# mit-acl/rl_collision_avoidance

Hardware: AMD Instinct MI355X
Metric: agent-steps/sec (env.step) at 4 agents x 8192 worlds per GPU (higher is better)
Workload: dtype f64

## Files before the change

### include/cavoid.h

```cpp
#ifndef CAVOID_H
#define CAVOID_H
#include <stdint.h>

#ifdef __cplusplus
extern "C" {
#endif

#define CAVOID_ABI_VERSION 3
#define CAVOID_MAX_ACTIONS 32
#define CAVOID_MAX_AGENTS 64

#define CAVOID_F_AT_GOAL 0x01u
#define CAVOID_F_RAN_OUT 0x02u
#define CAVOID_F_IN_COLL 0x04u
#define CAVOID_F_WAS_AT_GOAL 0x08u
#define CAVOID_F_WAS_IN_COLL 0x10u
#define CAVOID_F_PRESENT 0x20u
#define CAVOID_F_LEARNING 0x40u
#define CAVOID_F_POLICY_SHIFT 8
#define CAVOID_F_POLICY_MASK 7u
enum { CAVOID_POLICY_EXTERNAL = 0, CAVOID_POLICY_STATIC = 1, CAVOID_POLICY_NONCOOP = 2, CAVOID_POLICY_RVO = 3, CAVOID_POLICY_FROZEN_NET = 4 };
#define CAVOID_F_DONE_MASK 0x07u

enum { CAVOID_SORT_CLOSEST_LAST = 0, CAVOID_SORT_CLOSEST_FIRST = 1, CAVOID_SORT_TIME_TO_IMPACT = 2 };
// ... 95 lines not shown

enum {
    CAVOID_FORM_NONE = 0,
    CAVOID_FORM_STEP = 1,
    CAVOID_FORM_QUAD = 2,
    CAVOID_FORM_RVO = 3,
    CAVOID_FORM_LOOP_PF = 4,
    CAVOID_FORM_LOOP = 5,
    CAVOID_FORM_PIPE = 6,
    CAVOID_FORM_RELAY = 7,
    CAVOID_FORM_CROWD = 8,
    CAVOID_FORM_CROWD_RVO = 9
};
int32_t cavoid_last_step_form(const cavoid_env *env, int32_t *relay_consumers);

int cavoid_step_continuous_autoreset(cavoid_env *env, const float *actions , float *obs, float *rewards, uint8_t *done,
                                     uint8_t *game_over, void *stream);
int cavoid_step_continuous_autoreset_n(cavoid_env *env, const float *actions, int64_t action_stride, int32_t n_steps, int64_t out_step_stride,
                                       float *obs, float *rewards, uint8_t *done, uint8_t *game_over, void *stream);

int32_t cavoid_packed_width(const cavoid_env *env);
int cavoid_reset_packed(cavoid_env *env, const uint8_t *world_mask, float *packed, void *stream);
int cavoid_observe_packed(cavoid_env *env, float *packed, void *stream);
int cavoid_step_packed(cavoid_env *env, const int32_t *actions, float *packed, uint8_t *game_over, void *stream);
int cavoid_step_autoreset_packed(cavoid_env *env, const int32_t *actions, int64_t action_stride, int32_t n_steps, int64_t out_step_stride,
                                 float *packed, uint8_t *game_over, void *stream);
int cavoid_step_continuous_autoreset_packed(cavoid_env *env, const float *actions, int64_t action_stride, int32_t n_steps,
                                            int64_t out_step_stride, float *packed, uint8_t *game_over, void *stream);

typedef struct cavoid_comm cavoid_comm;
// ... 133 lines not shown
```

### rl_collision_avoidance_amd/_lib.py

```python
from __future__ import annotations

import ctypes as C
import os

from .build import LIB_PATH as _DEFAULT_LIB_PATH

LIB_PATH = os.environ.get("CAVOID_LIB", _DEFAULT_LIB_PATH)

MAX_ACTIONS = 32
MAX_AGENTS = 64
TILE_MAX_AGENTS = 16
RVO_WAVE = 2
ABI_VERSION = 3

F_AT_GOAL, F_RAN_OUT, F_IN_COLL, F_WAS_AT_GOAL, F_WAS_IN_COLL, F_PRESENT, F_LEARNING = 1, 2, 4, 8, 16, 32, 64
F_POLICY_SHIFT = 8
F_POLICY_MASK = 7
POLICY_EXTERNAL, POLICY_STATIC, POLICY_NONCOOP, POLICY_RVO, POLICY_FROZEN_NET = 0, 1, 2, 3, 4
F_DONE_MASK = 7
COMM_FORCE_RCCL = 1
STEP_FORMS = ("NONE", "STEP", "QUAD", "RVO", "LOOP_PF", "LOOP", "PIPE", "RELAY", "CROWD", "CROWD_RVO")


class CavoidCfg(C.Structure):
# ... 54 lines not shown
        self.code = code


_P = C.c_void_p
SYMBOLS = [
    ("cavoid_abi_version", C.c_int, []),
    ("cavoid_strerror", C.c_char_p, [C.c_int]),
    ("cavoid_last_hip_error", C.c_int, []),
    ("cavoid_default_cfg", C.c_int, [C.POINTER(CavoidCfg), C.c_int32, C.c_int32]),
    ("cavoid_default_actions", C.c_int, [_P, C.POINTER(C.c_int32)]),
    ("cavoid_create", C.c_int, [C.POINTER(CavoidCfg), C.c_int64, C.c_int64, C.c_int, C.POINTER(_P)]),
    ("cavoid_destroy", None, [_P]),
    ("cavoid_num_worlds", C.c_int64, [_P]),
    ("cavoid_obs_width", C.c_int32, [_P]),
    ("cavoid_last_step_form", C.c_int32, [_P, C.POINTER(C.c_int32)]),
    ("cavoid_seed", C.c_int, [_P, C.c_uint64, _P, _P]),
    ("cavoid_get_episode", C.c_int, [_P, _P, _P]),
    ("cavoid_pool_refresh", C.c_int, [_P, C.c_uint32, _P]),
    ("cavoid_set_state", C.c_int, [_P, _P, _P, _P, _P]),
    ("cavoid_get_state", C.c_int, [_P, _P, _P, _P, _P]),
    ("cavoid_reset", C.c_int, [_P, _P, _P, _P]),
    ("cavoid_observe", C.c_int, [_P, _P, _P]),
    ("cavoid_step", C.c_int, [_P, _P, _P, _P, _P, _P, _P]),
    ("cavoid_step_continuous", C.c_int, [_P, _P, _P, _P, _P, _P, _P]),
    ("cavoid_step_autoreset", C.c_int, [_P, _P, _P, _P, _P, _P, _P]),
    ("cavoid_step_autoreset_n", C.c_int, [_P, _P, C.c_int64, C.c_int32, C.c_int64, _P, _P, _P, _P, _P]),
    ("cavoid_step_continuous_autoreset", C.c_int, [_P, _P, _P, _P, _P, _P, _P]),
    ("cavoid_step_continuous_autoreset_n", C.c_int, [_P, _P, C.c_int64, C.c_int32, C.c_int64, _P, _P, _P, _P, _P]),
    ("cavoid_step_continuous_autoreset_packed", C.c_int, [_P, _P, C.c_int64, C.c_int32, C.c_int64, _P, _P, _P]),
    ("cavoid_step_autoreset_n_timed", C.c_int, [_P, _P, C.c_int64, C.c_int32, C.c_int32, C.c_int64, _P, _P, _P, _P, _P, C.POINTER(C.c_float)]),
# ... 77 lines not shown
```

### rl_collision_avoidance_amd/batched_env.py

```python
from __future__ import annotations

import ctypes as C
from typing import Optional, Tuple

import numpy as np
import torch

from . import _lib
from .config import EnvConfig

_SORT = {"closest_last": 0, "closest_first": 1, "time_to_impact": 2}
_DYN = {"unicycle": 0, "unicycle_max_turn_rate": 1, "holonomic": 2}


def make_cfg(config: Optional[EnvConfig] = None, **overrides) -> _lib.CavoidCfg:
    config = config or EnvConfig()
    cfg = _lib.CavoidCfg()
    N = int(config.MAX_NUM_AGENTS_IN_ENVIRONMENT)
    M = int(config.MAX_NUM_OTHER_AGENTS_OBSERVED)
    _lib.check(_lib.lib().cavoid_default_cfg(C.byref(cfg), N, M), "cavoid_default_cfg")
    cfg.dt = config.DT
    cfg.near_goal_threshold = config.NEAR_GOAL_THRESHOLD
    cfg.max_time_ratio = config.MAX_TIME_RATIO
    cfg.collision_dist = config.COLLISION_DIST
# ... 181 lines not shown
    def refresh_pool(self, epoch: int) -> None:
        _lib.check(self._lib.cavoid_pool_refresh(self._h, int(epoch) & 0xFFFFFFFF, self._stream()), "cavoid_pool_refresh")

    @property
    def episode(self) -> torch.Tensor:
        out = torch.empty((self.num_worlds,), dtype=torch.int32, device=self.device)
        _lib.check(self._lib.cavoid_get_episode(self._h, self._ptr(out), self._stream()), "cavoid_get_episode")
        return out

    @property
    def last_step_form(self) -> Tuple[str, int]:
        nc = C.c_int32(0)
        form = self._lib.cavoid_last_step_form(self._h, C.byref(nc))
        return _lib.STEP_FORMS[form], int(nc.value)

    def set_state(self, state_f64: torch.Tensor, state_f32: torch.Tensor, flags: torch.Tensor) -> None:
        A = self.num_worlds * self.max_agents
        f64 = self._want(state_f64, (4, A), torch.float64, "state_f64")
        f32 = self._want(state_f32, (5, A), torch.float32, "state_f32")
        fl = self._want(flags, (A,), torch.int32, "flags")
        _lib.check(self._lib.cavoid_set_state(self._h, self._ptr(f64), self._ptr(f32), self._ptr(fl), self._stream()),
                   "cavoid_set_state")

    def get_state(self) -> Tuple[torch.Tensor, torch.Tensor, torch.Tensor]:
        A = self.num_worlds * self.max_agents
        f64 = torch.empty((4, A), dtype=torch.float64, device=self.device)
        f32 = torch.empty((5, A), dtype=torch.float32, device=self.device)
        fl = torch.empty((A,), dtype=torch.int32, device=self.device)
        _lib.check(self._lib.cavoid_get_state(self._h, self._ptr(f64), self._ptr(f32), self._ptr(fl), self._stream()),
                   "cavoid_get_state")
# ... 164 lines not shown
```

### rl_collision_avoidance_amd/csrc/cavoid_capi.hip

```cpp
#include <hip/hip_runtime.h>
#include <hip/hip_ext.h>

#include <cmath>
#include <cstdlib>
#include <cstring>
#include <new>

#include "cavoid.h"
#include "cavoid_host.hpp"
#include "cavoid_kernels.hpp"
#include "cavoid_launch.hpp"
#include "cavoid_crowd.hpp"

using namespace cavoid;

thread_local int g_last_hip_error = 0;

extern "C" int cavoid_abi_version(void) { return CAVOID_ABI_VERSION; }

extern "C" int cavoid_last_hip_error(void) { return g_last_hip_error; }

extern "C" const char *cavoid_strerror(int code) {
    switch (code) {
        case CAVOID_OK: return "ok";
// ... 313 lines not shown
        return cavoid_launch_rvo(e, MODE, io, s, ev_start, ev_stop);
    if (MODE == MODE_STEP_AUTORESET) {
        const int rc = cavoid_launch_quad(e, io, s, ev_start, ev_stop);
        if (rc != CAVOID_EUNSUPPORTED) return rc;
    }
    const int rc = launch_on<MODE>(e, e->k, e->st, e->grid, io, s, ev_start, ev_stop);
    return stepping ? note_form(e, rc, CAVOID_FORM_STEP) : rc;
}

extern "C" int32_t cavoid_last_step_form(const cavoid_env *e, int32_t *relay_consumers) {
    const int32_t form = e ? e->last_form : CAVOID_FORM_NONE;
    if (relay_consumers) *relay_consumers = form == CAVOID_FORM_RELAY ? e->last_relay_consumers : 0;
    return form;
}

int cavoid_ahead_prepare(cavoid_env *e, int32_t n_steps, hipStream_t s, hipEvent_t *timed_start) {
    if (!e || e->ahead_R <= 0) return CAVOID_OK;
    if (n_steps + 1 > e->ahead_R) return CAVOID_EUNSUPPORTED;
    hipStreamCaptureStatus cap = hipStreamCaptureStatusNone;
    (void)hipStreamIsCapturing(s, &cap);
    const bool capturing = cap != hipStreamCaptureStatusNone;
    if (capturing) e->ahead_always = true;
    if (!e->ahead_always && e->ahead_primed && e->ahead_budget >= n_steps + 1) return CAVOID_OK;
    const int64_t waves = (e->W + e->k.wpw - 1) / e->k.wpw;
    const bool in_place = e->ahead_always;
    const dim3 grid((unsigned)((waves + 3) / 4), in_place ? 1u : (e->ahead_primed ? 4u : 32u)), block(256);
    const uint32_t *hi_in = e->ahead_hi[e->ahead_cur];
    uint32_t *hi_out = e->ahead_hi[in_place ? e->ahead_cur : (e->ahead_cur ^ 1)];
    hipEvent_t ev_fill = (timed_start && !capturing) ? *timed_start : nullptr;
    if (ev_fill) *timed_start = nullptr;
    const int rc = dispatch_n(e->cfg.max_agents, EnvNs{}, [&](auto n) -> int {
        launch_kernel(ahead_fill_kernel<decltype(n)::value>, grid, block, 0, s, ev_fill, nullptr, e->k, e->st.episode, hi_in, hi_out, e->pool, e->ahead_R);
        return CAVOID_OK;
    });
    if (rc != CAVOID_OK) return rc;
    HIP_TRY(hipGetLastError());
    if (!in_place) e->ahead_cur ^= 1;
    if (!capturing) { e->ahead_primed = true; e->ahead_budget = e->ahead_R; }
    return CAVOID_OK;
}
void cavoid_ahead_consumed(cavoid_env *e, int32_t n_steps) {
    if (!e || e->ahead_R <= 0) return;
    e->ahead_budget = e->ahead_budget > n_steps ? e->ahead_budget - n_steps : 0;
}

static int fill_pool(cavoid_env *e, hipStream_t s) {
    if (e->ahead_R > 0) {
        e->ahead_budget = 0;
        e->ahead_primed = false;
        HIP_TRY(hipMemsetAsync(e->ahead_hi[0], 0xFF, 2 * (size_t)e->W * sizeof(uint32_t), s));
        return CAVOID_OK;
    }
    if (e->pool_size <= 0) return CAVOID_OK;
    HIP_TRY(hipMemsetAsync(e->pool_episode, 0xFF, (size_t)e->pool_size * sizeof(uint32_t), s));
    KCfg k = e->k;
    k.num_worlds = e->pool_size;
    k.world_offset = 0;
    k.pool_size = 0;
// ... 119 lines not shown
    return launch<MODE_STEP>(e, io, static_cast<hipStream_t>(stream));
}

static int launch_autoreset(cavoid_env *e, KIO io, const int32_t *actions, int64_t action_stride, int32_t n_steps, int64_t out_step_stride,
                            hipStream_t s, hipEvent_t ev_start = nullptr, hipEvent_t ev_stop = nullptr, const float *cont = nullptr) {
    if (e->cfg.dynamics == CAVOID_DYN_HOLONOMIC && !cont) return CAVOID_EINVAL;
    if (n_steps < 1 || action_stride < 0) return CAVOID_EINVAL;
    if (cont && n_steps > 1 && action_stride != 0 && action_stride < 2 * e->A) return CAVOID_EINVAL;
    if (out_step_stride != 0 && out_step_stride < e->W) return CAVOID_EINVAL;
    io.out_step_stride = n_steps > 1 ? out_step_stride : 0;
    io.actions = actions;
    io.cont = cont;
    io.action_stride = action_stride;
    io.n_steps = n_steps;
    e->last_form = CAVOID_FORM_NONE;
    if (int rc = cavoid_ahead_prepare(e, n_steps, s, &ev_start)) return rc;
    const int rc = (n_steps > 1 || e->prefetch_single)
                       ? cavoid_launch_multistep(e, io, e->latency_mode != 0, s, ev_start, ev_stop)
                       : launch<MODE_STEP_AUTORESET>(e, io, s, ev_start, ev_stop);
    cavoid_ahead_consumed(e, n_steps);
    return rc;
}

extern "C" int cavoid_step_autoreset(cavoid_env *e, const int32_t *actions, float *obs, float *rew, uint8_t *done, uint8_t *game_over, void *stream) {
    if (step_args(e, actions, rew, done, game_over) != CAVOID_OK) return CAVOID_EINVAL;
    return launch_autoreset(e, plain_io(e, obs, rew, done, game_over), actions, 0, 1, 0, static_cast<hipStream_t>(stream));
}

extern "C" int cavoid_step_autoreset_n(cavoid_env *e, const int32_t *actions, int64_t action_stride, int32_t n_steps, int64_t out_step_stride,
                                       float *obs, float *rew, uint8_t *done, uint8_t *game_over, void *stream) {
    if (step_args(e, actions, rew, done, game_over) != CAVOID_OK || n_steps < 0) return CAVOID_EINVAL;
    if (n_steps == 0) return CAVOID_OK;
    return launch_autoreset(e, plain_io(e, obs, rew, done, game_over), actions, action_stride, n_steps, out_step_stride,
                            static_cast<hipStream_t>(stream));
}
// ... 118 lines not shown
```

### rl_collision_avoidance_amd/csrc/cavoid_kernels.hpp

```cpp
#pragma once
#include <hip/hip_runtime.h>
#include <stdint.h>

#include "cavoid.h"

namespace cavoid {

#ifdef CAVOID_TRACE
__device__ unsigned long long *g_trace = nullptr;
#define CAVOID_STAMP(k)                                                                \
    do {                                                                               \
        if (lane == 0 && g_trace) g_trace[wave * 16 + (k)] = (unsigned long long)clock64(); \
    } while (0)
#else
#define CAVOID_STAMP(k) do { } while (0)
#endif

#define CAVOID_RARE(x) __builtin_expect(!!(x), 0)
#ifndef CAVOID_SKIP
#define CAVOID_SKIP 0
#endif

constexpr double kPi = 3.14159265358979323846;
constexpr int kTileMaxAgents = 16;
// ... 53 lines not shown

struct KIO {
    PoolRec *pool_out;
    const int32_t *actions;
    const float *cont;
    const uint8_t *mask;
    float *obs;
    float *rew;
    uint8_t *done;
    uint8_t *game_over;
    int64_t action_stride;
    int64_t out_step_stride;
    int32_t n_steps;
    int32_t obs_stride;
    int32_t packed;
};

__device__ __forceinline__ double wrap_closed_fixup(double a, uint32_t switches) {
    if (CAVOID_RARE(switches & kSwWrapClosed)) a = a == -kPi ? kPi : a;
    return a;
}
__device__ __forceinline__ double wrap_angle(double a, uint32_t switches) {
    a = a >= kPi ? a - 2.0 * kPi : a;
    a = a < -kPi ? a + 2.0 * kPi : a;
    if (CAVOID_RARE(__ballot(a >= kPi || a < -kPi) != 0ull)) {
        while (a >= kPi) a -= 2.0 * kPi;
        while (a < -kPi) a += 2.0 * kPi;
    }
    return wrap_closed_fixup(a, switches);
}
// ... 684 lines not shown
    a.gx = r.gx; a.gy = r.gy; a.radius = r.radius; a.pref = r.pref;
    a.flags = r.flags;
    a.vx = a.vy = 0.0;
    a.speed = 0.0f;
}

template <int N>
__device__ __forceinline__ void new_episode(const KCfg &c, const PoolRec *pool, uint32_t gw, uint32_t ep, int i, Agent &a) {
    if (c.pool_size > 0) {
        load_pool(pool, (int64_t)pool_index(c, gw, ep) * N + i, a);
    } else {
        generate_agent<N>(c, gw, ep, i, a);
    }
}

template <int N>
__device__ __forceinline__ void ahead_fill_wave(const KCfg &c, const uint32_t *episode, const uint32_t *hi_in, uint32_t *hi_out, PoolRec *ahead, const int need,
                                                const int64_t wave, const int lane, const int y, const int ny, double *sc_d, float *sc_r) {
    const int wpw = c.wpw, lanes_used = wpw * N;
    const int lw = lane / N, i = lane - lw * N;
    const int64_t w = wave * wpw + lw;
    const bool active = lane < lanes_used && w < c.num_worlds;
    const int base = lane < lanes_used ? lw * N : 0;
    uint32_t ep = 0u, fh = 0u;
    if (active) {
        ep = episode[w];
        fh = hi_in[w];
        if (fh == 0xFFFFFFFFu || (int32_t)(fh - ep) < 0) fh = ep;
    }
    const uint32_t target = ep + (uint32_t)need;
    int missing = active ? (int)(int32_t)(target - fh) : 0;
    missing = missing < 0 ? 0 : missing;
    int trips = missing;
#pragma unroll
    for (int o = 32; o > 0; o >>= 1) { const int v = __shfl_xor(trips, o, 64); trips = v > trips ? v : trips; }
    const uint32_t gw = (uint32_t)(c.world_offset + w);
    for (int k = y; k < trips; k += ny) {
        const uint32_t e = fh + 1u + (uint32_t)k;
        const bool fresh = active && k < missing;
        Agent a;
        absent_agent(a);
        if (c.gen_mode == 1) generate_world_v2<N>(c, gw, e, i, base, lane, fresh, sc_d, sc_d + 64, sc_d + 128, sc_d + 192, sc_r, a);
        else if (fresh) generate_agent<N>(c, gw, e, i, a);
        if (fresh) {
            PoolRec r;
            r.px = a.px; r.py = a.py; r.heading = a.heading; r.t_rem = a.t_rem;
            r.gx = a.gx; r.gy = a.gy; r.radius = a.radius; r.pref = a.pref;
            r.flags = a.flags; r.pad[0] = r.pad[1] = r.pad[2] = 0u;
            ahead[((int64_t)w * c.ahead + (int64_t)(e & (uint32_t)(c.ahead - 1))) * N + i] = r;
        }
    }
    if (active && i == 0 && y == 0) hi_out[w] = missing > 0 ? target : fh;
}

template <int N>
__global__ void __launch_bounds__(256) ahead_fill_kernel(const KCfg c, const uint32_t *episode, const uint32_t *hi_in, uint32_t *hi_out, PoolRec *ahead, const int need) {
    __shared__ double sh_d[4][4 * 64];
    __shared__ float sh_r[4][64];
    const int wave_in_block = threadIdx.x >> 6;
    ahead_fill_wave<N>(c, episode, hi_in, hi_out, ahead, need, (int64_t)blockIdx.x * 4 + wave_in_block, threadIdx.x & 63, (int)blockIdx.y, (int)gridDim.y,
                       sh_d[wave_in_block], sh_r[wave_in_block]);
}

constexpr double kRvoEps = 1e-5;
__device__ __forceinline__ double det2(double ax, double ay, double bx, double by) { return ax * by - ay * bx; }

struct Line { double px, py, dx, dy; };
// ... 731 lines not shown
```

### rl_collision_avoidance_amd/csrc/cavoid_launch.hpp

```cpp
#pragma once
#include <hip/hip_runtime.h>
#include <hip/hip_ext.h>

#include <type_traits>

#include "cavoid.h"
#include "cavoid_host.hpp"
#include "cavoid_kernels.hpp"

struct cavoid_env {
    int device = 0;
    int64_t W = 0, A = 0, world_offset = 0;
    cavoid_cfg cfg{};
    cavoid::KCfg k{};
    cavoid::KState st{};
    cavoid::PoolRec *pool = nullptr;
    uint32_t *pool_episode = nullptr;
    int64_t pool_size = 0;
    int ahead_R = 0;
    uint32_t *ahead_hi[2] = {nullptr, nullptr};
    int ahead_cur = 0;
    int ahead_budget = 0;
    bool ahead_primed = false;
    bool ahead_always = false;
    void *slab = nullptr;
    void *pool_slab = nullptr;
    double *d_actions = nullptr;
    int waves_per_block = 4;
    int grid = 0;
    int pipeline = 2;
    int relay_consumers = 3;
    int latency_mode = 0;
    int quad = -1;
    int prefetch_single = 0;
    int last_form = CAVOID_FORM_NONE;
    int last_relay_consumers = 0;
    hipEvent_t ev0 = nullptr, ev1 = nullptr;
};

// ... 80 lines not shown
    const dim3 grid((unsigned)tiles), block(128);
    const int rc = dispatch_n(e->cfg.max_agents, EnvNs{}, [&](auto n) -> int {
        constexpr int N = decltype(n)::value;
        const size_t lds = pipe_lds_fixed_bytes<N>() + tail;
        if (lds > 65536) return CAVOID_EUNSUPPORTED;
        launch_kernel(env_pipe_kernel<N, RVO>, grid, block, lds, s, ev_start, ev_stop, k, e->st, e->pool, io);
        return CAVOID_OK;
    });
    if (rc != CAVOID_OK) return rc;
    HIP_TRY(hipGetLastError());
    return CAVOID_OK;
}

}

int cavoid_ahead_prepare(cavoid_env *e, int32_t n_steps, hipStream_t s, hipEvent_t *timed_start = nullptr);
void cavoid_ahead_consumed(cavoid_env *e, int32_t n_steps);
int cavoid_launch_relay(cavoid_env *e, const cavoid::KIO &io, hipStream_t s, hipEvent_t ev_start, hipEvent_t ev_stop);
int cavoid_launch_quad(cavoid_env *e, const cavoid::KIO &io, hipStream_t s, hipEvent_t ev_start, hipEvent_t ev_stop);
int cavoid_launch_multistep(cavoid_env *e, const cavoid::KIO &io, bool prefetch, hipStream_t s, hipEvent_t ev_start, hipEvent_t ev_stop);
int cavoid_launch_rvo(cavoid_env *e, int mode, const cavoid::KIO &io, hipStream_t s, hipEvent_t ev_start, hipEvent_t ev_stop);
int cavoid_launch_crowd(cavoid_env *e, int mode, const cavoid::KCfg &k, const cavoid::KState &st, int64_t worlds, const cavoid::KIO &io,
                        hipStream_t s, hipEvent_t ev_start, hipEvent_t ev_stop);
int cavoid_launch_crowd_rvo(cavoid_env *e, int mode, const cavoid::KCfg &k, const cavoid::KState &st, int64_t worlds, const cavoid::KIO &io,
                            hipStream_t s, hipEvent_t ev_start, hipEvent_t ev_stop);
static inline int crowd_step_form(const cavoid_env *e) { return e->k.rvo_enabled ? CAVOID_FORM_CROWD_RVO : CAVOID_FORM_CROWD; }
#ifdef CAVOID_TRACE
int cavoid_debug_trace_multistep(unsigned long long *dev_ptr);
int cavoid_debug_trace_rvo(unsigned long long *dev_ptr);
int cavoid_debug_trace_relay(unsigned long long *dev_ptr);
int cavoid_debug_trace_quad(unsigned long long *dev_ptr);
#endif
```

### rl_collision_avoidance_amd/csrc/cavoid_multistep.hip

```cpp
#include "cavoid_launch.hpp"

using namespace cavoid;

int cavoid_launch_multistep(cavoid_env *e, const KIO &io, bool prefetch, hipStream_t s, hipEvent_t ev_start, hipEvent_t ev_stop) {
    if (crowd_form(e->cfg.max_agents))
        return note_form(e, cavoid_launch_crowd(e, MODE_STEP_AUTORESET_N, e->k, e->st, e->W, io, s, ev_start, ev_stop), crowd_step_form(e));
    if (e->k.rvo_enabled || (e->k.gen_mode == 1 && e->k.pool_size <= 0))
        return cavoid_launch_rvo(e, prefetch ? MODE_STEP_AUTORESET_PF : MODE_STEP_AUTORESET_N, io, s, ev_start, ev_stop);
    if (prefetch && e->pipeline >= 2 && !io.cont) {
        const int rc = cavoid_launch_relay(e, io, s, ev_start, ev_stop);
        if (rc != CAVOID_EUNSUPPORTED) return rc;
    }
    if (prefetch && e->pipeline && !io.cont) {
        const int rc = launch_pipe<false>(e, io, s, ev_start, ev_stop);
        if (rc != CAVOID_EUNSUPPORTED) return note_form(e, rc, CAVOID_FORM_PIPE);
    }
    if (prefetch) return note_form(e, launch_on<MODE_STEP_AUTORESET_PF>(e, e->k, e->st, e->grid, io, s, ev_start, ev_stop), CAVOID_FORM_LOOP_PF);
    return note_form(e, launch_on<MODE_STEP_AUTORESET_N>(e, e->k, e->st, e->grid, io, s, ev_start, ev_stop), CAVOID_FORM_LOOP);
}

#ifdef CAVOID_TRACE
int cavoid_debug_trace_multistep(unsigned long long *dev_ptr) { return set_trace(dev_ptr); }
#endif
```

### rl_collision_avoidance_amd/csrc/cavoid_relay.hip

```cpp
#include "cavoid_launch.hpp"
#include "cavoid_relay.hpp"

using namespace cavoid;

template <int N>
static int relay_allow_lds() {
    static bool allowed = false;
    if (!allowed) {
        HIP_TRY(hipFuncSetAttribute(reinterpret_cast<const void *>(env_relay_kernel<N>), hipFuncAttributeMaxDynamicSharedMemorySize, (int)kRelayLdsLimit));
        allowed = true;
    }
    return CAVOID_OK;
}

int cavoid_launch_relay(cavoid_env *e, const KIO &io, hipStream_t s, hipEvent_t ev_start, hipEvent_t ev_stop) {
    const KCfg &k = e->k;
    if (k.rvo_enabled || k.pool_size <= 0 || !io.obs || !io.actions || io.cont) return CAVOID_EUNSUPPORTED;
    if (k.switches & kSwSkipDonePairs) return CAVOID_EUNSUPPORTED;
    const int64_t tiles = (e->W + k.wpw - 1) / k.wpw;
    if (tiles > 512) return CAVOID_EUNSUPPORTED;
    if (e->cfg.max_agents > kRelayMaxAgents) return CAVOID_EUNSUPPORTED;
    const int row = io.obs_stride;
    const int tile_floats = (k.tile_rows * row + 3) & ~3;
    if (k.tile_rows < k.wpw * e->cfg.max_agents) return CAVOID_EUNSUPPORTED;
    const dim3 grid((unsigned)tiles);
    int used_nc = 0;
    const int rc = dispatch_n(e->cfg.max_agents, RelayNs{}, [&](auto n) -> int {
        constexpr int N = decltype(n)::value;
        int nc = e->relay_consumers;
        while (nc > 1 && relay_lds_fixed_bytes<N>() + (size_t)nc * tile_floats * sizeof(float) > kRelayLdsLimit) --nc;
        const size_t lds = relay_lds_fixed_bytes<N>() + (size_t)nc * tile_floats * sizeof(float);
        if (lds > kRelayLdsLimit || (nc < 2 && e->relay_consumers >= 2)) return CAVOID_EUNSUPPORTED;
        if (lds > 65536) {
            const int rc_opt = relay_allow_lds<N>();
            if (rc_opt != CAVOID_OK) return rc_opt;
        }
        used_nc = nc;
        launch_kernel(env_relay_kernel<N>, grid, dim3(64 * (3 + nc)), lds, s, ev_start, ev_stop, k, e->st, e->pool, io);
        return CAVOID_OK;
    });
    if (rc != CAVOID_OK) return rc;
    HIP_TRY(hipGetLastError());
    return note_form(e, CAVOID_OK, CAVOID_FORM_RELAY, used_nc);
}

#ifdef CAVOID_TRACE
int cavoid_debug_trace_relay(unsigned long long *dev_ptr) { return set_trace(dev_ptr); }
#endif
```

### rl_collision_avoidance_amd/csrc/cavoid_relay.hpp

```cpp
#pragma once
#include "cavoid_kernels.hpp"

namespace cavoid {

constexpr int kRelayMaxAgents = 6;
template <int N>
__host__ __device__ constexpr int relay_ring() { return N <= 5 ? 8 : 4; }
constexpr size_t kRelayLdsLimit = 80 * 1024;
constexpr int kRelayActRing = 64;
constexpr int kRelayActAhead = 48;
constexpr int kRelayEvq = 8;

struct RelaySeq {
    int spec;
    int stage;
    int res;
    int fin;
    int act;
    int ev;
    int nxt;
    int cons[kRelayMaxConsumers];
    int cfin[kRelayMaxConsumers];
    int coop[2];
    int kernarg[2];
    int tile_id;
};
static_assert(sizeof(RelaySeq) % 16 == 0, "the event queue behind it holds 64-bit masks; the tiles further on are read 16 bytes at a time");
struct RelayTent { double px[64], py[64], vx[64], vy[64], heading[64]; float r[64], gx[64], gy[64], pref[64]; uint32_t flags[64]; };
struct RelayRes { uint32_t flags[64], ctl[64]; float rew[64]; };
struct RelayNxt { double px[64], py[64], heading[64], t_rem[64]; float gx[64], gy[64], radius[64], pref[64]; uint32_t flags[64]; };
#ifndef CAVOID_RELAY_ORDER
#define CAVOID_RELAY_ORDER 0x432150
#endif
#ifndef CAVOID_RELAY_PRIO_D
#define CAVOID_RELAY_PRIO_D 3
#endif
#ifndef CAVOID_RELAY_PRIO_P
#define CAVOID_RELAY_PRIO_P 3
#endif
#ifndef CAVOID_RELAY_PRIO_L
#define CAVOID_RELAY_PRIO_L 0
#endif
#ifndef CAVOID_RELAY_PRIO_C
#define CAVOID_RELAY_PRIO_C 1
#endif
#ifndef CAVOID_RELAY_ABL
#define CAVOID_RELAY_ABL 0
#endif
__device__ __forceinline__ int relay_role_of(int wv, int NC) {
    if (NC == 3) return (int)(((unsigned)CAVOID_RELAY_ORDER >> (4 * wv)) & 15u);
    return wv;
}
constexpr int kRelayCoopWaves = 3;
constexpr int kRelayCoopFromN = 4;
template <int N>
struct RelayCoop {
    static constexpr int K = Others<N>::K;
    uint64_t key[K][64];
    uint32_t bits[K][64];
// ... 197 lines not shown
#endif
        uint32_t lo = orderable((float)(ry * e.tx - rx * e.ty));
        if (SW) {
            if (c.switches & kSwIndexTie) lo = (uint32_t)other_index(st.i, o, N);
            if (c.switches & kSwExactGap) { lo = 0u; hi = 0x7FFFFFFEu - (orderable((float)gap_o) >> 1); }
        }
        hi = seen ? hi : kKeySentinel + (uint32_t)o;
        co.key[o][lane] = ((uint64_t)hi << 32) | lo;
        co.bits[o][lane] = seen ? 2u : 0u;
        gapf[o] = (float)gap_o;
        neighbour_features(e, (float)e.prll_x, (float)e.prll_y, rx, ry, q, feat[o]);
    }
}

struct RelayArgs { KCfg c; KState s; const PoolRec *pool; KIO io; };
template <class T>
__device__ __forceinline__ void relay_load_args(T &dst, const __attribute__((address_space(4))) T *src) {
    static_assert(sizeof(T) % 4 == 0, "whole words");
    const __attribute__((address_space(4))) uint32_t *w = (const __attribute__((address_space(4))) uint32_t *)src;
    uint32_t d[sizeof(T) / 4];
#pragma unroll
    for (int k = 0; k < (int)(sizeof(T) / 4); ++k) d[k] = w[k];
    __builtin_memcpy(&dst, d, sizeof(T));
}
template <int N>
__device__ __forceinline__ void relay_coop_last(unsigned char *smem) {
    unsigned char *sp = smem + lds_floats_block() * sizeof(float);
    RelaySeq *seq = reinterpret_cast<RelaySeq *>(sp); sp += sizeof(RelaySeq) + kRelayEvq * sizeof(unsigned long long);
    const unsigned long long kp = (unsigned long long)(uint32_t)relay_peek(&seq->kernarg[0]) | ((unsigned long long)(uint32_t)relay_peek(&seq->kernarg[1]) << 32);
    typedef const __attribute__((address_space(4))) RelayArgs *ArgP;
    const ArgP ka = (ArgP)kp;
    KCfg c;
    KIO io;
    relay_load_args(c, &ka->c);
    relay_load_args(io, &ka->io);
    RelayTent *tents = reinterpret_cast<RelayTent *>(sp); sp += relay_ring<N>() * sizeof(RelayTent) + sizeof(RelayNxt);
    RelayRes *ress = reinterpret_cast<RelayRes *>(sp); sp += relay_ring<N>() * sizeof(RelayRes) + kRelayActRing * 64;
    RelayCoop<N> *coopb = reinterpret_cast<RelayCoop<N> *>(sp); sp += relay_coop_bytes<N>();
    float *tiles = reinterpret_cast<float *>(sp);
    const int lane0 = threadIdx.x & 63;
    const int NC = (blockDim.x >> 6) - 3;
    const int role = relay_role_of(threadIdx.x >> 6, NC);
    const int pw = role < 2 ? role : 2;
    const int ostride = io.obs_stride;
    const int tile_floats = (c.tile_rows * ostride + 3) & ~3;
    const int wpw = c.wpw, lanes_used = wpw * N;
    const int64_t wave = relay_peek(&seq->tile_id);
    const int64_t w0 = wave * wpw;
    const int lw = lane0 / N, i0 = lane0 - lw * N;
    const int64_t w = w0 + lw;
    const bool active = lane0 < lanes_used && w < c.num_worlds;
    const int base0 = lane0 < lanes_used ? lw * N : 0;
    const int64_t a_idx0 = w * N + i0;
    const bool packed = io.packed != 0;
    int64_t worlds_here = c.num_worlds - w0;
    if (worlds_here > wpw) worlds_here = wpw;
    if (worlds_here < 0) worlds_here = 0;
    const int n_steps = io.n_steps;
    constexpr int K = Others<N>::K;
    const int t = n_steps - 1;
    const int cid_l = t % NC;
    float *tile = tiles + (size_t)cid_l * tile_floats;
// ... 51 lines not shown
        if (io.out_step_stride != 0 && lines) flush_tile<4, true, true>(tile, dst, rows_active * ostride, pw * 64 + lane0, 64 * kRelayCoopWaves);
        else if (io.out_step_stride != 0) flush_tile<4, true>(tile, dst, rows_active * ostride, pw * 64 + lane0, 64 * kRelayCoopWaves);
        else flush_tile<4>(tile, dst, rows_active * ostride, pw * 64 + lane0, 64 * kRelayCoopWaves);
    }
    if (pw == 0 && active) {
        if (!packed) {
            io.rew[slot_w * N + a_idx0] = rew_c;
            io.done[slot_w * N + a_idx0] = (ctl_c & 1u) ? 1 : 0;
        }
        if (i0 == 0) io.game_over[slot_w + w] = (ctl_c & 2u) ? 1 : 0;
    }
    if (pw == 0) RELAY_MARK(29);
}

template <int N>
__global__ void __launch_bounds__(64 * (3 + kRelayMaxConsumers), 1) env_relay_kernel(const KCfg c, const KState s, const PoolRec *pool, const KIO io) {
    extern __shared__ __attribute__((aligned(16))) unsigned char smem[];
    unsigned char *sp = smem;
    double *lds_tab = reinterpret_cast<double *>(sp); sp += lds_floats_block() * sizeof(float);
    RelaySeq *seq = reinterpret_cast<RelaySeq *>(sp); sp += sizeof(RelaySeq);
    unsigned long long *evq = reinterpret_cast<unsigned long long *>(sp); sp += kRelayEvq * sizeof(unsigned long long);
    RelayTent *tents = reinterpret_cast<RelayTent *>(sp); sp += relay_ring<N>() * sizeof(RelayTent);
    RelayNxt *nbuf = reinterpret_cast<RelayNxt *>(sp); sp += sizeof(RelayNxt);
    RelayRes *ress = reinterpret_cast<RelayRes *>(sp); sp += relay_ring<N>() * sizeof(RelayRes);
    unsigned char *actring = sp; sp += kRelayActRing * 64;
    RelayCoop<N> *coopb = reinterpret_cast<RelayCoop<N> *>(sp); sp += relay_coop_bytes<N>();
    float *tiles = reinterpret_cast<float *>(sp);

    const int NC = (blockDim.x >> 6) - 3;
    const int role = relay_role_of(threadIdx.x >> 6, NC);
    const int lane0 = threadIdx.x & 63;
    const int ostride = io.obs_stride;
    const int tile_floats = (c.tile_rows * ostride + 3) & ~3;
    const int wpw = c.wpw, lanes_used = wpw * N;
    const int64_t wave = blockIdx.x;
    const int64_t w0 = wave * wpw;
    const int lw = lane0 / N, i0 = lane0 - lw * N;
    const int64_t w = w0 + lw;
    const bool active = lane0 < lanes_used && w < c.num_worlds;
    const int base0 = lane0 < lanes_used ? lw * N : 0;
    const int64_t a_idx0 = w * N + i0;
    const bool packed = io.packed != 0;
    int64_t worlds_here = c.num_worlds - w0;
    if (worlds_here > wpw) worlds_here = wpw;
    if (worlds_here < 0) worlds_here = 0;
    const int n_steps = io.n_steps;
    constexpr bool kCoop = N >= kRelayCoopFromN;
    const bool coop_role = role < 2 || role == 2 + NC;

    if (role == 0 && lane0 < (int)(sizeof(RelaySeq) / sizeof(int))) reinterpret_cast<int *>(seq)[lane0] = 0;
    if constexpr (kCoop) {
        if (role == 0 && lane0 == 0) {
            const unsigned long long kp = (unsigned long long)__builtin_amdgcn_kernarg_segment_ptr();
            seq->kernarg[0] = (int)(uint32_t)kp; seq->kernarg[1] = (int)(uint32_t)(kp >> 32);
            seq->tile_id = (int)blockIdx.x;
        }
    }

    if (role == 0) {
        __builtin_amdgcn_s_setprio(CAVOID_RELAY_PRIO_D);
        RELAY_MARK(20);
        KCfg cd = c;
        asm volatile("" : "+s"(cd.dt), "+s"(cd.near_goal_sq), "+s"(cd.actions_fp32), "+s"(cd.dynamics),
                     "+s"(cd.timeout_enabled), "+s"(cd.switches));
        const RelayTrig trig = relay_trig_constants();
        Agent a;
        a.px = a.py = a.heading = a.t_rem = a.vx = a.vy = 0.0;
        a.gx = a.gy = a.radius = a.pref = a.speed = 0.0f;
        a.flags = 0u;
        uint32_t episode = 0u;
// ... 273 lines not shown
                continue;
            }
            if (loaded < n_steps && loaded < fin + kRelayActAhead) {
                int upto = fin + kRelayActAhead;
                if (upto > loaded + 8) upto = loaded + 8;
                if (upto > n_steps) upto = n_steps;
                load_actions(upto);
                idle_polls = 0;
                relay_post(&seq->act, loaded);
                continue;
            }
            if (fin >= n_steps && relay_peek(&seq->stage) > n_steps) break;
            if (++idle_polls > kRelayPollLimit) __builtin_trap();
            __builtin_amdgcn_s_sleep(2);
        }
    } else {
        __builtin_amdgcn_s_setprio(CAVOID_RELAY_PRIO_C);
        KCfg cc = c;
        asm volatile("" : "+s"(cc.switches));
        const int cid = role - 2;
        float *tile = tiles + (size_t)cid * tile_floats;
        __syncthreads();
        const int n_mine = kCoop ? n_steps - 1 : n_steps;
        for (int t = cid; t < n_mine; t += NC) {
            int lane = lane0, i = i0, base = base0;
            asm volatile("" : "+v"(lane), "+v"(i), "+v"(base));
            RELAY_STAMP(16);
            relay_wait_bounded(&seq->fin, t + 1);
            RELAY_STAMP(17);
            if (CAVOID_RELAY_ABL & 1) { relay_post(&seq->cons[cid], t + 1); continue; }
// ... 35 lines not shown
                if (i0 == 0) io.game_over[slot_w + w] = (ctl_c & 2u) ? 1 : 0;
            }
            relay_post(&seq->cons[cid], t + 1);
            RELAY_STAMP(19);
            if (t == 0) RELAY_MARK(28);
            if (t == n_steps - 1) RELAY_MARK(29);
        }
        __builtin_amdgcn_s_waitcnt(0);
        if (cid == 0) RELAY_MARK(30);
        relay_post(&seq->cfin[cid], 1);
    }
    if constexpr (kCoop) {
        if (coop_role) relay_coop_last<N>(smem);
    }
}

}
```

Before: 23.49 billion.

## Fold lookahead pool refill into relay kernel as an extra low-priority wave

Adds a top-up wave role to the relay kernel that refills the per-world lookahead episode ring while the step pipeline runs. The host then skips the separate ahead-prepare refill launch whenever the relay form can absorb it. The goal is to remove a separate kernel launch and its serialization before each multistep call. In exchange each block carries one more wave, and launch bounds change so that more blocks per CU may fit for small N, which can alter register allocation. It also adds device-specific LDS attribute caching and refill counters for introspection.

```diff
diff --git a/include/cavoid.h b/include/cavoid.h
--- a/include/cavoid.h
+++ b/include/cavoid.h
@@ -133,6 +133,8 @@
 };
 int32_t cavoid_last_step_form(const cavoid_env *env, int32_t *relay_consumers);
 
+int cavoid_ahead_info(const cavoid_env *env, int64_t *refill_launches, int32_t *budget);
+
 int cavoid_step_continuous_autoreset(cavoid_env *env, const float *actions , float *obs, float *rewards, uint8_t *done,
                                      uint8_t *game_over, void *stream);
 int cavoid_step_continuous_autoreset_n(cavoid_env *env, const float *actions, int64_t action_stride, int32_t n_steps, int64_t out_step_stride,
diff --git a/rl_collision_avoidance_amd/_lib.py b/rl_collision_avoidance_amd/_lib.py
--- a/rl_collision_avoidance_amd/_lib.py
+++ b/rl_collision_avoidance_amd/_lib.py
@@ -92,6 +92,7 @@
     ("cavoid_num_worlds", C.c_int64, [_P]),
     ("cavoid_obs_width", C.c_int32, [_P]),
     ("cavoid_last_step_form", C.c_int32, [_P, C.POINTER(C.c_int32)]),
+    ("cavoid_ahead_info", C.c_int, [_P, C.POINTER(C.c_int64), C.POINTER(C.c_int32)]),
     ("cavoid_seed", C.c_int, [_P, C.c_uint64, _P, _P]),
     ("cavoid_get_episode", C.c_int, [_P, _P, _P]),
     ("cavoid_pool_refresh", C.c_int, [_P, C.c_uint32, _P]),
diff --git a/rl_collision_avoidance_amd/batched_env.py b/rl_collision_avoidance_amd/batched_env.py
--- a/rl_collision_avoidance_amd/batched_env.py
+++ b/rl_collision_avoidance_amd/batched_env.py
@@ -219,6 +219,12 @@
         form = self._lib.cavoid_last_step_form(self._h, C.byref(nc))
         return _lib.STEP_FORMS[form], int(nc.value)
 
+    @property
+    def lookahead_info(self) -> Tuple[int, int]:
+        refills, budget = C.c_int64(0), C.c_int32(0)
+        _lib.check(self._lib.cavoid_ahead_info(self._h, C.byref(refills), C.byref(budget)), "cavoid_ahead_info")
+        return int(refills.value), int(budget.value)
+
     def set_state(self, state_f64: torch.Tensor, state_f32: torch.Tensor, flags: torch.Tensor) -> None:
         A = self.num_worlds * self.max_agents
         f64 = self._want(state_f64, (4, A), torch.float64, "state_f64")
diff --git a/rl_collision_avoidance_amd/csrc/cavoid_capi.hip b/rl_collision_avoidance_amd/csrc/cavoid_capi.hip
--- a/rl_collision_avoidance_amd/csrc/cavoid_capi.hip
+++ b/rl_collision_avoidance_amd/csrc/cavoid_capi.hip
@@ -351,9 +351,10 @@
     return form;
 }
 
-int cavoid_ahead_prepare(cavoid_env *e, int32_t n_steps, hipStream_t s, hipEvent_t *timed_start) {
+int cavoid_ahead_prepare(cavoid_env *e, int32_t n_steps, hipStream_t s, hipEvent_t *timed_start, bool relay_topup) {
     if (!e || e->ahead_R <= 0) return CAVOID_OK;
     if (n_steps + 1 > e->ahead_R) return CAVOID_EUNSUPPORTED;
+    if (relay_topup && e->ahead_primed && e->ahead_budget >= n_steps) return CAVOID_OK;
     hipStreamCaptureStatus cap = hipStreamCaptureStatusNone;
     (void)hipStreamIsCapturing(s, &cap);
     const bool capturing = cap != hipStreamCaptureStatusNone;
@@ -372,13 +373,22 @@
     });
     if (rc != CAVOID_OK) return rc;
     HIP_TRY(hipGetLastError());
+    e->ahead_refills += 1;
     if (!in_place) e->ahead_cur ^= 1;
     if (!capturing) { e->ahead_primed = true; e->ahead_budget = e->ahead_R; }
     return CAVOID_OK;
 }
-void cavoid_ahead_consumed(cavoid_env *e, int32_t n_steps) {
+void cavoid_ahead_consumed(cavoid_env *e, int32_t n_steps, bool relay_topup) {
     if (!e || e->ahead_R <= 0) return;
-    e->ahead_budget = e->ahead_budget > n_steps ? e->ahead_budget - n_steps : 0;
+    if (relay_topup) e->ahead_budget = e->ahead_R - n_steps;
+    else e->ahead_budget = e->ahead_budget > n_steps ? e->ahead_budget - n_steps : 0;
+}
+
+extern "C" int cavoid_ahead_info(const cavoid_env *e, int64_t *refill_launches, int32_t *budget) {
+    if (!e) return CAVOID_EINVAL;
+    if (refill_launches) *refill_launches = e->ahead_refills;
+    if (budget) *budget = e->ahead_R > 0 && e->ahead_primed ? e->ahead_budget : 0;
+    return CAVOID_OK;
 }
 
 static int fill_pool(cavoid_env *e, hipStream_t s) {
@@ -528,11 +538,14 @@
     io.action_stride = action_stride;
     io.n_steps = n_steps;
     e->last_form = CAVOID_FORM_NONE;
-    if (int rc = cavoid_ahead_prepare(e, n_steps, s, &ev_start)) return rc;
-    const int rc = (n_steps > 1 || e->prefetch_single)
-                       ? cavoid_launch_multistep(e, io, e->latency_mode != 0, s, ev_start, ev_stop)
-                       : launch<MODE_STEP_AUTORESET>(e, io, s, ev_start, ev_stop);
-    cavoid_ahead_consumed(e, n_steps);
+    const bool loop = n_steps > 1 || e->prefetch_single;
+    const bool topup = loop && e->ahead_R > 0 && relay_form_first(e, io, e->latency_mode != 0) && cavoid_relay_takes_topup(e, io, s);
+    if (int rc = cavoid_ahead_prepare(e, n_steps, s, &ev_start, topup)) return rc;
+    if (topup) io.ahead_hi = e->ahead_hi[e->ahead_cur];
+    const int rc = loop ? cavoid_launch_multistep(e, io, e->latency_mode != 0, s, ev_start, ev_stop)
+                        : launch<MODE_STEP_AUTORESET>(e, io, s, ev_start, ev_stop);
+    if (topup && rc != CAVOID_OK) { e->ahead_primed = false; e->ahead_budget = 0; }
+    else cavoid_ahead_consumed(e, n_steps, topup);
     return rc;
 }
 
diff --git a/rl_collision_avoidance_amd/csrc/cavoid_kernels.hpp b/rl_collision_avoidance_amd/csrc/cavoid_kernels.hpp
--- a/rl_collision_avoidance_amd/csrc/cavoid_kernels.hpp
+++ b/rl_collision_avoidance_amd/csrc/cavoid_kernels.hpp
@@ -91,6 +91,7 @@
     int32_t n_steps;
     int32_t obs_stride;
     int32_t packed;
+    uint32_t *ahead_hi;
 };
 
 __device__ __forceinline__ double wrap_closed_fixup(double a, uint32_t switches) {
@@ -805,6 +806,35 @@
     }
 }
 
+template <int N, bool V1_ONLY = false>
+__device__ __forceinline__ void ahead_fill_range(const KCfg &c, const uint32_t ep, uint32_t fh, const bool active, const int64_t w, const int i, const int base,
+                                                 const int lane, uint32_t *hi_out, PoolRec *ahead, const int need, const int y, const int ny, double *sc_d,
+                                                 float *sc_r) {
+    if (active && (fh == 0xFFFFFFFFu || (int32_t)(fh - ep) < 0)) fh = ep;
+    const uint32_t target = ep + (uint32_t)need;
+    int missing = active ? (int)(int32_t)(target - fh) : 0;
+    missing = missing < 0 ? 0 : missing;
+    int trips = missing;
+#pragma unroll
+    for (int o = 32; o > 0; o >>= 1) { const int v = __shfl_xor(trips, o, 64); trips = v > trips ? v : trips; }
+    const uint32_t gw = (uint32_t)(c.world_offset + w);
+    for (int k = y; k < trips; k += ny) {
+        const uint32_t e = fh + 1u + (uint32_t)k;
+        const bool fresh = active && k < missing;
+        Agent a;
+        absent_agent(a);
+        if (!V1_ONLY && c.gen_mode == 1) generate_world_v2<N>(c, gw, e, i, base, lane, fresh, sc_d, sc_d + 64, sc_d + 128, sc_d + 192, sc_r, a);
+        else if (fresh) generate_agent<N>(c, gw, e, i, a);
+        if (fresh) {
+            PoolRec r;
+            r.px = a.px; r.py = a.py; r.heading = a.heading; r.t_rem = a.t_rem;
+            r.gx = a.gx; r.gy = a.gy; r.radius = a.radius; r.pref = a.pref;
+            r.flags = a.flags; r.pad[0] = r.pad[1] = r.pad[2] = 0u;
+            ahead[((int64_t)w * c.ahead + (int64_t)(e & (uint32_t)(c.ahead - 1))) * N + i] = r;
+        }
+    }
+    if (active && i == 0 && y == 0) hi_out[w] = missing > 0 ? target : fh;
+}
 template <int N>
 __device__ __forceinline__ void ahead_fill_wave(const KCfg &c, const uint32_t *episode, const uint32_t *hi_in, uint32_t *hi_out, PoolRec *ahead, const int need,
                                                 const int64_t wave, const int lane, const int y, const int ny, double *sc_d, float *sc_r) {
@@ -817,31 +847,8 @@
     if (active) {
         ep = episode[w];
         fh = hi_in[w];
-        if (fh == 0xFFFFFFFFu || (int32_t)(fh - ep) < 0) fh = ep;
-    }
-    const uint32_t target = ep + (uint32_t)need;
-    int missing = active ? (int)(int32_t)(target - fh) : 0;
-    missing = missing < 0 ? 0 : missing;
-    int trips = missing;
-#pragma unroll
-    for (int o = 32; o > 0; o >>= 1) { const int v = __shfl_xor(trips, o, 64); trips = v > trips ? v : trips; }
-    const uint32_t gw = (uint32_t)(c.world_offset + w);
-    for (int k = y; k < trips; k += ny) {
-        const uint32_t e = fh + 1u + (uint32_t)k;
-        const bool fresh = active && k < missing;
-        Agent a;
-        absent_agent(a);
-        if (c.gen_mode == 1) generate_world_v2<N>(c, gw, e, i, base, lane, fresh, sc_d, sc_d + 64, sc_d + 128, sc_d + 192, sc_r, a);
-        else if (fresh) generate_agent<N>(c, gw, e, i, a);
-        if (fresh) {
-            PoolRec r;
-            r.px = a.px; r.py = a.py; r.heading = a.heading; r.t_rem = a.t_rem;
-            r.gx = a.gx; r.gy = a.gy; r.radius = a.radius; r.pref = a.pref;
-            r.flags = a.flags; r.pad[0] = r.pad[1] = r.pad[2] = 0u;
-            ahead[((int64_t)w * c.ahead + (int64_t)(e & (uint32_t)(c.ahead - 1))) * N + i] = r;
-        }
-    }
-    if (active && i == 0 && y == 0) hi_out[w] = missing > 0 ? target : fh;
+    }
+    ahead_fill_range<N>(c, ep, fh, active, w, i, base, lane, hi_out, ahead, need, y, ny, sc_d, sc_r);
 }
 
 template <int N>
diff --git a/rl_collision_avoidance_amd/csrc/cavoid_launch.hpp b/rl_collision_avoidance_amd/csrc/cavoid_launch.hpp
--- a/rl_collision_avoidance_amd/csrc/cavoid_launch.hpp
+++ b/rl_collision_avoidance_amd/csrc/cavoid_launch.hpp
@@ -23,6 +23,10 @@
     int ahead_budget = 0;
     bool ahead_primed = false;
     bool ahead_always = false;
+    int64_t ahead_refills = 0;
+    int relay_topup_nc = -1;
+    size_t relay_topup_lds = 0;
+    bool relay_topup_fits = false;
     void *slab = nullptr;
     void *pool_slab = nullptr;
     double *d_actions = nullptr;
@@ -133,9 +137,14 @@
 
 }
 
-int cavoid_ahead_prepare(cavoid_env *e, int32_t n_steps, hipStream_t s, hipEvent_t *timed_start = nullptr);
-void cavoid_ahead_consumed(cavoid_env *e, int32_t n_steps);
+int cavoid_ahead_prepare(cavoid_env *e, int32_t n_steps, hipStream_t s, hipEvent_t *timed_start = nullptr, bool relay_topup = false);
+void cavoid_ahead_consumed(cavoid_env *e, int32_t n_steps, bool relay_topup = false);
 int cavoid_launch_relay(cavoid_env *e, const cavoid::KIO &io, hipStream_t s, hipEvent_t ev_start, hipEvent_t ev_stop);
+static inline bool relay_form_first(const cavoid_env *e, const cavoid::KIO &io, bool prefetch) {
+    return !cavoid::crowd_form(e->cfg.max_agents) && !e->k.rvo_enabled && !(e->k.gen_mode == 1 && e->k.pool_size <= 0) && prefetch && e->pipeline >= 2 &&
+           !io.cont;
+}
+bool cavoid_relay_takes_topup(cavoid_env *e, const cavoid::KIO &io, hipStream_t s);
 int cavoid_launch_quad(cavoid_env *e, const cavoid::KIO &io, hipStream_t s, hipEvent_t ev_start, hipEvent_t ev_stop);
 int cavoid_launch_multistep(cavoid_env *e, const cavoid::KIO &io, bool prefetch, hipStream_t s, hipEvent_t ev_start, hipEvent_t ev_stop);
 int cavoid_launch_rvo(cavoid_env *e, int mode, const cavoid::KIO &io, hipStream_t s, hipEvent_t ev_start, hipEvent_t ev_stop);
diff --git a/rl_collision_avoidance_amd/csrc/cavoid_multistep.hip b/rl_collision_avoidance_amd/csrc/cavoid_multistep.hip
--- a/rl_collision_avoidance_amd/csrc/cavoid_multistep.hip
+++ b/rl_collision_avoidance_amd/csrc/cavoid_multistep.hip
@@ -3,14 +3,16 @@
 using namespace cavoid;
 
 int cavoid_launch_multistep(cavoid_env *e, const KIO &io, bool prefetch, hipStream_t s, hipEvent_t ev_start, hipEvent_t ev_stop) {
+    if (relay_form_first(e, io, prefetch)) {
+        const int rc = cavoid_launch_relay(e, io, s, ev_start, ev_stop);
+        if (rc != CAVOID_EUNSUPPORTED || io.ahead_hi) return rc;
+    } else if (io.ahead_hi) {
+        return CAVOID_EINVAL;
+    }
     if (crowd_form(e->cfg.max_agents))
         return note_form(e, cavoid_launch_crowd(e, MODE_STEP_AUTORESET_N, e->k, e->st, e->W, io, s, ev_start, ev_stop), crowd_step_form(e));
     if (e->k.rvo_enabled || (e->k.gen_mode == 1 && e->k.pool_size <= 0))
         return cavoid_launch_rvo(e, prefetch ? MODE_STEP_AUTORESET_PF : MODE_STEP_AUTORESET_N, io, s, ev_start, ev_stop);
-    if (prefetch && e->pipeline >= 2 && !io.cont) {
-        const int rc = cavoid_launch_relay(e, io, s, ev_start, ev_stop);
-        if (rc != CAVOID_EUNSUPPORTED) return rc;
-    }
     if (prefetch && e->pipeline && !io.cont) {
         const int rc = launch_pipe<false>(e, io, s, ev_start, ev_stop);
         if (rc != CAVOID_EUNSUPPORTED) return note_form(e, rc, CAVOID_FORM_PIPE);
diff --git a/rl_collision_avoidance_amd/csrc/cavoid_relay.hip b/rl_collision_avoidance_amd/csrc/cavoid_relay.hip
--- a/rl_collision_avoidance_amd/csrc/cavoid_relay.hip
+++ b/rl_collision_avoidance_amd/csrc/cavoid_relay.hip
@@ -3,17 +3,56 @@
 
 using namespace cavoid;
 
+constexpr int kRelayMaxDevices = 64;
 template <int N>
 static int relay_allow_lds() {
-    static bool allowed = false;
-    if (!allowed) {
-        HIP_TRY(hipFuncSetAttribute(reinterpret_cast<const void *>(env_relay_kernel<N>), hipFuncAttributeMaxDynamicSharedMemorySize, (int)kRelayLdsLimit));
-        allowed = true;
+    static bool allowed[kRelayMaxDevices] = {};
+    int dev = 0;
+    HIP_TRY(hipGetDevice(&dev));
+    const bool cached = dev >= 0 && dev < kRelayMaxDevices;
+    if (cached && allowed[dev]) return CAVOID_OK;
+    if (hipFuncSetAttribute(reinterpret_cast<const void *>(env_relay_kernel<N>), hipFuncAttributeMaxDynamicSharedMemorySize, (int)kRelayLdsLimit) != hipSuccess) {
+        (void)hipGetLastError();
+        return CAVOID_EUNSUPPORTED;
+    }
+    if (cached) allowed[dev] = true;
+    return CAVOID_OK;
+}
+
+struct RelayShape {
+    int nc = 0;
+    size_t lds = 0;
+    bool topup = false;
+};
+template <int N>
+static int relay_shape_n(cavoid_env *e, int tile_floats, bool want_topup, RelayShape &sh) {
+    int nc = e->relay_consumers;
+    while (nc > 1 && relay_lds_fixed_bytes<N>() + (size_t)nc * tile_floats * sizeof(float) > kRelayLdsLimit) --nc;
+    const size_t lds = relay_lds_fixed_bytes<N>() + (size_t)nc * tile_floats * sizeof(float);
+    if (lds > kRelayLdsLimit || (nc < 2 && e->relay_consumers >= 2)) return CAVOID_EUNSUPPORTED;
+    if (lds > 65536) {
+        const int rc_opt = relay_allow_lds<N>();
+        if (rc_opt != CAVOID_OK) return rc_opt;
+    }
+    sh.nc = nc;
+    sh.lds = lds;
+    sh.topup = false;
+    if (want_topup && e->k.gen_mode == 0) {
+        if (e->relay_topup_nc != nc || e->relay_topup_lds != lds) {
+            int blocks = 0;
+            if (hipOccupancyMaxActiveBlocksPerMultiprocessor(&blocks, reinterpret_cast<const void *>(env_relay_kernel<N>), 64 * (4 + nc), lds) != hipSuccess) {
+                (void)hipGetLastError();
+                blocks = 0;
+            }
+            e->relay_topup_nc = nc;
+            e->relay_topup_lds = lds;
+            e->relay_topup_fits = blocks >= 2;
+        }
+        sh.topup = e->relay_topup_fits;
     }
     return CAVOID_OK;
 }
-
-int cavoid_launch_relay(cavoid_env *e, const KIO &io, hipStream_t s, hipEvent_t ev_start, hipEvent_t ev_stop) {
+static int relay_shape(cavoid_env *e, const KIO &io, bool want_topup, RelayShape &sh) {
     const KCfg &k = e->k;
     if (k.rvo_enabled || k.pool_size <= 0 || !io.obs || !io.actions || io.cont) return CAVOID_EUNSUPPORTED;
     if (k.switches & kSwSkipDonePairs) return CAVOID_EUNSUPPORTED;
@@ -23,25 +62,35 @@
     const int row = io.obs_stride;
     const int tile_floats = (k.tile_rows * row + 3) & ~3;
     if (k.tile_rows < k.wpw * e->cfg.max_agents) return CAVOID_EUNSUPPORTED;
-    const dim3 grid((unsigned)tiles);
-    int used_nc = 0;
+    return dispatch_n(e->cfg.max_agents, RelayNs{}, [&](auto n) -> int { return relay_shape_n<decltype(n)::value>(e, tile_floats, want_topup, sh); });
+}
+
+static bool relay_wants_topup(const cavoid_env *e, hipStream_t s) {
+    if (e->ahead_R <= 0 || e->ahead_always || e->k.gen_mode != 0) return false;
+    hipStreamCaptureStatus cap = hipStreamCaptureStatusNone;
+    (void)hipStreamIsCapturing(s, &cap);
+    return cap == hipStreamCaptureStatusNone;
+}
+
+bool cavoid_relay_takes_topup(cavoid_env *e, const KIO &io, hipStream_t s) {
+    RelayShape sh;
+    return relay_wants_topup(e, s) && relay_shape(e, io, true, sh) == CAVOID_OK && sh.topup;
+}
+
+int cavoid_launch_relay(cavoid_env *e, const KIO &io, hipStream_t s, hipEvent_t ev_start, hipEvent_t ev_stop) {
+    RelayShape sh;
+    const int rc_shape = relay_shape(e, io, io.ahead_hi != nullptr, sh);
+    if (rc_shape != CAVOID_OK) return rc_shape;
+    if ((io.ahead_hi != nullptr) != sh.topup) return CAVOID_EINVAL;
+    const int64_t tiles = (e->W + e->k.wpw - 1) / e->k.wpw;
+    const dim3 grid((unsigned)tiles), block(64 * (3 + sh.nc + (sh.topup ? 1 : 0)));
     const int rc = dispatch_n(e->cfg.max_agents, RelayNs{}, [&](auto n) -> int {
-        constexpr int N = decltype(n)::value;
-        int nc = e->relay_consumers;
-        while (nc > 1 && relay_lds_fixed_bytes<N>() + (size_t)nc * tile_floats * sizeof(float) > kRelayLdsLimit) --nc;
-        const size_t lds = relay_lds_fixed_bytes<N>() + (size_t)nc * tile_floats * sizeof(float);
-        if (lds > kRelayLdsLimit || (nc < 2 && e->relay_consumers >= 2)) return CAVOID_EUNSUPPORTED;
-        if (lds > 65536) {
-            const int rc_opt = relay_allow_lds<N>();
-            if (rc_opt != CAVOID_OK) return rc_opt;
-        }
-        used_nc = nc;
-        launch_kernel(env_relay_kernel<N>, grid, dim3(64 * (3 + nc)), lds, s, ev_start, ev_stop, k, e->st, e->pool, io);
+        launch_kernel(env_relay_kernel<decltype(n)::value>, grid, block, sh.lds, s, ev_start, ev_stop, e->k, e->st, e->pool, io);
         return CAVOID_OK;
     });
     if (rc != CAVOID_OK) return rc;
     HIP_TRY(hipGetLastError());
-    return note_form(e, CAVOID_OK, CAVOID_FORM_RELAY, used_nc);
+    return note_form(e, CAVOID_OK, CAVOID_FORM_RELAY, sh.nc);
 }
 
 #ifdef CAVOID_TRACE
diff --git a/rl_collision_avoidance_amd/csrc/cavoid_relay.hpp b/rl_collision_avoidance_amd/csrc/cavoid_relay.hpp
--- a/rl_collision_avoidance_amd/csrc/cavoid_relay.hpp
+++ b/rl_collision_avoidance_amd/csrc/cavoid_relay.hpp
@@ -1,4 +1,7 @@
 #pragma once
+#include <cstddef>
+#include <type_traits>
+
 #include "cavoid_kernels.hpp"
 
 namespace cavoid {
@@ -10,6 +13,7 @@
 constexpr int kRelayActRing = 64;
 constexpr int kRelayActAhead = 48;
 constexpr int kRelayEvq = 8;
+constexpr int kRelayTopupMaxN = 5;
 
 struct RelaySeq {
     int spec;
@@ -30,7 +34,7 @@
 struct RelayRes { uint32_t flags[64], ctl[64]; float rew[64]; };
 struct RelayNxt { double px[64], py[64], heading[64], t_rem[64]; float gx[64], gy[64], radius[64], pref[64]; uint32_t flags[64]; };
 #ifndef CAVOID_RELAY_ORDER
-#define CAVOID_RELAY_ORDER 0x432150
+#define CAVOID_RELAY_ORDER 0x6432150
 #endif
 #ifndef CAVOID_RELAY_PRIO_D
 #define CAVOID_RELAY_PRIO_D 3
@@ -43,6 +47,9 @@
 #endif
 #ifndef CAVOID_RELAY_PRIO_C
 #define CAVOID_RELAY_PRIO_C 1
+#endif
+#ifndef CAVOID_RELAY_PRIO_T
+#define CAVOID_RELAY_PRIO_T 0
 #endif
 #ifndef CAVOID_RELAY_ABL
 #define CAVOID_RELAY_ABL 0
@@ -270,6 +277,13 @@
 }
 
 struct RelayArgs { KCfg c; KState s; const PoolRec *pool; KIO io; };
+static_assert(alignof(KCfg) == 8 && alignof(KState) == 8 && alignof(KIO) == 8 && alignof(RelayArgs) == 8, "kernel arguments: 8-byte aligned");
+static_assert(sizeof(KCfg) % 8 == 0 && sizeof(KState) % 8 == 0 && sizeof(KIO) % 8 == 0, "kernel arguments: whole 8-byte words, no tail padding to skip");
+static_assert(offsetof(RelayArgs, c) == 0 && offsetof(RelayArgs, s) == sizeof(KCfg) && offsetof(RelayArgs, pool) == sizeof(KCfg) + sizeof(KState) &&
+                  offsetof(RelayArgs, io) == sizeof(KCfg) + sizeof(KState) + sizeof(const PoolRec *) &&
+                  sizeof(RelayArgs) == sizeof(KCfg) + sizeof(KState) + sizeof(const PoolRec *) + sizeof(KIO),
+              "RelayArgs must be the kernel's argument segment, argument by argument");
+static_assert(sizeof(KIO) == 104 && offsetof(KIO, n_steps) == 80 && offsetof(KIO, ahead_hi) == 96, "KIO changed: check what relay_coop_last reads from it");
 template <class T>
 __device__ __forceinline__ void relay_load_args(T &dst, const __attribute__((address_space(4))) T *src) {
     static_assert(sizeof(T) % 4 == 0, "whole words");
@@ -295,13 +309,14 @@
     RelayCoop<N> *coopb = reinterpret_cast<RelayCoop<N> *>(sp); sp += relay_coop_bytes<N>();
     float *tiles = reinterpret_cast<float *>(sp);
     const int lane0 = threadIdx.x & 63;
-    const int NC = (blockDim.x >> 6) - 3;
+    const int tile_nc = relay_peek(&seq->tile_id);
+    const int NC = tile_nc >> 16;
     const int role = relay_role_of(threadIdx.x >> 6, NC);
     const int pw = role < 2 ? role : 2;
     const int ostride = io.obs_stride;
     const int tile_floats = (c.tile_rows * ostride + 3) & ~3;
     const int wpw = c.wpw, lanes_used = wpw * N;
-    const int64_t wave = relay_peek(&seq->tile_id);
+    const int64_t wave = tile_nc & 0xFFFF;
     const int64_t w0 = wave * wpw;
     const int lw = lane0 / N, i0 = lane0 - lw * N;
     const int64_t w = w0 + lw;
@@ -383,7 +398,37 @@
 }
 
 template <int N>
-__global__ void __launch_bounds__(64 * (3 + kRelayMaxConsumers), 1) env_relay_kernel(const KCfg c, const KState s, const PoolRec *pool, const KIO io) {
+__device__ __forceinline__ void relay_topup() {
+    __builtin_amdgcn_s_setprio(CAVOID_RELAY_PRIO_T);
+    unsigned long long kp = (unsigned long long)__builtin_amdgcn_kernarg_segment_ptr();
+    asm volatile("" : "+s"(kp));
+    typedef const __attribute__((address_space(4))) RelayArgs *ArgP;
+    const ArgP ka = (ArgP)kp;
+    KCfg c;
+    uint32_t *episode, *hi;
+    const PoolRec *ring;
+    relay_load_args(c, &ka->c);
+    relay_load_args(episode, &ka->s.episode);
+    relay_load_args(ring, &ka->pool);
+    relay_load_args(hi, &ka->io.ahead_hi);
+    const int lane0 = threadIdx.x & 63;
+    const int wpw = c.wpw, lanes_used = wpw * N;
+    const int lw = lane0 / N, i0 = lane0 - lw * N;
+    const int64_t w = (int64_t)blockIdx.x * wpw + lw;
+    const bool active = lane0 < lanes_used && w < c.num_worlds;
+    const int base0 = lane0 < lanes_used ? lw * N : 0;
+    uint32_t ep = 0u, fh = 0u;
+    if (active) {
+        ep = episode[w];
+        fh = hi[w];
+    }
+    asm volatile("" : "+v"(ep), "+v"(fh));
+    __syncthreads();
+    ahead_fill_range<N, true>(c, ep, fh, active, w, i0, base0, lane0, hi, const_cast<PoolRec *>(ring), c.ahead, 0, 1, nullptr, nullptr);
+}
+
+template <int N>
+__global__ void __launch_bounds__(64 * (4 + kRelayMaxConsumers), N <= kRelayTopupMaxN ? 4 : 1) env_relay_kernel(const KCfg c, const KState s, const PoolRec *pool, const KIO io) {
     extern __shared__ __attribute__((aligned(16))) unsigned char smem[];
     unsigned char *sp = smem;
     double *lds_tab = reinterpret_cast<double *>(sp); sp += lds_floats_block() * sizeof(float);
@@ -396,7 +441,7 @@
     RelayCoop<N> *coopb = reinterpret_cast<RelayCoop<N> *>(sp); sp += relay_coop_bytes<N>();
     float *tiles = reinterpret_cast<float *>(sp);
 
-    const int NC = (blockDim.x >> 6) - 3;
+    const int NC = (blockDim.x >> 6) - 3 - (io.ahead_hi ? 1 : 0);
     const int role = relay_role_of(threadIdx.x >> 6, NC);
     const int lane0 = threadIdx.x & 63;
     const int ostride = io.obs_stride;
@@ -422,7 +467,7 @@
         if (role == 0 && lane0 == 0) {
             const unsigned long long kp = (unsigned long long)__builtin_amdgcn_kernarg_segment_ptr();
             seq->kernarg[0] = (int)(uint32_t)kp; seq->kernarg[1] = (int)(uint32_t)(kp >> 32);
-            seq->tile_id = (int)blockIdx.x;
+            seq->tile_id = (int)blockIdx.x | (NC << 16);
         }
     }
 
@@ -726,6 +771,8 @@
             if (++idle_polls > kRelayPollLimit) __builtin_trap();
             __builtin_amdgcn_s_sleep(2);
         }
+    } else if (role == 3 + NC) {
+        relay_topup<N>();
     } else {
         __builtin_amdgcn_s_setprio(CAVOID_RELAY_PRIO_C);
         KCfg cc = c;
@@ -791,5 +838,7 @@
         if (coop_role) relay_coop_last<N>(smem);
     }
 }
-
-}
+static_assert(std::is_same<decltype(&env_relay_kernel<4>), void (*)(const KCfg, const KState, const PoolRec *, const KIO)>::value,
+              "relay_coop_last reloads the kernel's arguments through RelayArgs: keep the two in step");
+
+}
```

New measurement: 23.83 billion (median of 6 runs). 1.01x the previous value.
